# cbouilla/spasm

Hardware: AMD Instinct MI355X
Metric: rows eliminated/sec (sparse Schur complement, mod 42013) (higher is better)
Workload: dtype i32 sums of i16 x i16 products

## Files before the change

spasm_amd/csrc/backsolve.hip:

```cpp
#include <algorithm>
#include <cinttypes>
#include <type_traits>
#include <thread>
#include <vector>

#include "device_types.h"
#include "field_dev.h"
#include "sgn_dev.h"

namespace sh {

int usable_cpus();

namespace {

constexpr int BS_RING = 768;
constexpr int BS_NEARCAP = 1024;
constexpr int BS_PASSCAP = 80;
constexpr int BS_PASSROWS = 32;
constexpr uint32_t BS_NONE = 0xFFFFFFFFu;

template <typename T> T *dalloc(int64_t count)
{
	return static_cast<T *>(sh::big_alloc((size_t) (count > 0 ? count : 1) * sizeof(T)));
// ... 1187 lines not shown
					dst[u] = at;
					if (v0[u] != 0)
						cbuf[at] = qq[u].x;
					if (v1[u] != 0)
						cbuf[at + (v0[u] != 0 ? 1u : 0u)] = qq[u].y;
					gpos += (uint32_t) (__popcll(m0) + __popcll(m1));
				}
				for (uint32_t t = lane; t < gpos; t += 64)
					oj[wpos + t] = cbuf[t];
#pragma unroll
				for (int u = 0; u < AP_TU; u++) {
					if (v0[u] != 0)
						cbuf[dst[u]] = v0[u];
					if (v1[u] != 0)
						cbuf[dst[u] + (v0[u] != 0 ? 1u : 0u)] = v1[u];
				}
				for (uint32_t t = lane; t < gpos; t += 64)
					ox[wpos + t] = cbuf[t];
				wpos += gpos;
			};
			constexpr int GW = 64 * AP_TU;
			issue(0, qa);
			issue(GW, qb);
			for (int t0 = 0; t0 < nwords; t0 += 3 * GW) {
				issue(t0 + 2 * GW, qc);
				emit(t0, qa);
				issue(t0 + 3 * GW, qa);
				if (t0 + GW < nwords)
					emit(t0 + GW, qb);
				issue(t0 + 4 * GW, qb);
				if (t0 + 2 * GW < nwords)
					emit(t0 + 2 * GW, qc);
			}
		}
		st_done += fits ? 1 : 0;
		k0 = k1;
		c0 = c1;
		k1 = -1;
		uint32_t *const t = x0;
		x0 = x1;
		x1 = t;
		return true;
	};

	for (;;) {
		if (k0 >= 0)
			settle(k1 >= 0);
		const int k = next_ticket(d, lane);
		if (k >= a.nrows)
			break;
		uint32_t *xw = (k0 < 0) ? x0 : x1;
		const int i = a.rows[k];
		const int64_t lo = a.Ap[i], hi = a.Ap[i + 1];
		st_input += (unsigned long long) (hi - lo);
		int count = s16_reduce_segment<true>(d, F, G, lo, hi, 0, nwords, plist, xw, lane, true, st_piv);
		if (count < 0) {
			count = 0;
			for (int t0 = 0; t0 < nwords; t0 += 64) {
				const uint32_t w = xw[t0 + lane];
				count += __popcll(__ballot((w & 0xFFFFu) != 0)) + __popcll(__ballot((w >> 16) != 0));
			}
		}
		if (lane == 0)
			__hip_atomic_store(&d.status[k], LB_FLAG_LEN | (unsigned long long) count, __ATOMIC_RELAXED, __HIP_MEMORY_SCOPE_AGENT);
		if (k0 < 0) {
			k0 = k;
			c0 = count;
		} else {
			k1 = k;
			c1 = count;
		}
	}
	while (k0 >= 0)
		settle(true);
	if (lane == 0) {
		if (lost)
			atomicOr(&a.ctr[CTR_STATUS], 4);
		atomicAdd(&a.ctr64[C64_INPUT], st_input);
		atomicAdd(&a.ctr64[C64_ELIM], st_piv);
		atomicAdd(&a.ctr[a.done_ctr], st_done);
	}
}

constexpr int SCAN_BLOCK = 1024;

__global__ __launch_bounds__(SCAN_BLOCK) void bs_scan_lengths_kernel(const int *len, int n, const unsigned long long *block_sum, int64_t *Sp, int64_t cap,
                                                                      int *ctr)
{
	__shared__ long long part[SCAN_BLOCK / 64];
	__shared__ long long s_base;
	const int tid = threadIdx.x, lane = tid & 63, wave = tid >> 6;
	const int g = blockIdx.x;
	auto wave_sum = [](long long v) -> long long {
		for (int sft = 32; sft >= 1; sft >>= 1) {
			const uint32_t lo32 = (uint32_t) __shfl_xor((int) (uint32_t) v, sft);
			const uint32_t hi32 = (uint32_t) __shfl_xor((int) (uint32_t) ((unsigned long long) v >> 32), sft);
			v += (long long) (((unsigned long long) hi32 << 32) | lo32);
		}
		return v;
	};
	long long before = 0;
	for (int b = tid; b < g; b += SCAN_BLOCK)
		before += (long long) block_sum[b];
	before = wave_sum(before);
	if (lane == 0)
		part[wave] = before;
	__syncthreads();
	if (tid == 0) {
		long long t = Sp[0];
		for (int w = 0; w < SCAN_BLOCK / 64; w++)
			t += part[w];
		s_base = t;
	}
	__syncthreads();
	const long long base = s_base;
	__syncthreads();
	const int k = g * SCAN_BLOCK + tid;
	const long long mine = (k < n) ? (long long) len[k] : 0;
	long long incl = mine;
	for (int sft = 1; sft < 64; sft <<= 1) {
		const uint32_t lo32 = (uint32_t) __shfl_up((int) (uint32_t) incl, sft);
		const uint32_t hi32 = (uint32_t) __shfl_up((int) (uint32_t) ((unsigned long long) incl >> 32), sft);
		if (lane >= sft)
			incl += (long long) (((unsigned long long) hi32 << 32) | lo32);
	}
	if (lane == 63)
		part[wave] = incl;
	__syncthreads();
	long long waves_before = 0;
	for (int w = 0; w < wave; w++)
		waves_before += part[w];
	const long long end = base + waves_before + incl;
	if (k < n) {
		Sp[k + 1] = end;
		if (k == n - 1 && end > cap)
			atomicOr(&ctr[CTR_STATUS], 1);
	}
}

struct ExpandArgs {
	const uint32_t *stage;
	int nwords, nrows;
	const int64_t *Sp;
	int *Sj, *Sx;
	int64_t cap;
	const int *q;
	SgnDev G;
};


template <int FMT> __global__ __launch_bounds__(256) void bs_expand_kernel(ExpandArgs e)
{
	constexpr int TU = 4;
	__shared__ int stage_j[4][128 * TU], stage_x[4][128 * TU];
	const int lane = threadIdx.x & 63, wv = threadIdx.x >> 6;
	const int wave = (int) ((blockIdx.x * blockDim.x + threadIdx.x) >> 6), nwaves = (int) ((gridDim.x * blockDim.x) >> 6);
	const int2 *q2 = reinterpret_cast<const int2 *>(e.q) + lane;
	const int *q1 = e.q + lane;
	const SgnDev G = e.G;
	const uint32_t pu = (uint32_t) G.p, halfu = (uint32_t) G.half;
	auto balanced = [&](uint32_t v) -> int { return (v > halfu) ? (int) (v - pu) : (int) v; };
	const int last = e.nwords - 64 * TU;
	int *sj = stage_j[wv], *sx = stage_x[wv];
	for (int k = wave; k < e.nrows; k += nwaves) {
		const int64_t off = e.Sp[k], end = e.Sp[k + 1];
		if (end > e.cap || end == off)
// ... 707 lines not shown
	}
	b.sparse_init = (B.nnp <= 4 * (int64_t) B.r && env_int("SPASM_HIP_BS_SPARSE_INIT", 1) != 0) ? 1 : 0;
	HIP_CHECK(hipEventRecord(B.ev0, stream));
	if (fresh || !b.sparse_init)
		HIP_CHECK(hipMemsetAsync(B.d_R, 0, bytes, stream));
	if (!b.sparse_init) {
		if (packed)
			hipLaunchKernelGGL(bs_init_kernel<uint16_t>, dim3((B.r + 255) / 256), dim3(256), 0, stream, b);
		else
			hipLaunchKernelGGL(bs_init_kernel<uint32_t>, dim3((B.r + 255) / 256), dim3(256), 0, stream, b);
	}
	const int shape = B.shape;
	if (shape == 3)
		snprintf(B.kernel_build, sizeof(B.kernel_build), "backsolve_kernel<true,true,8,8,true,768,64,31,2>");
	else if (shape == 4)
		snprintf(B.kernel_build, sizeof(B.kernel_build), "backsolve_kernel<true,true,10,10,true,1260,64,48,1>");
	else if (shape == 5)
		snprintf(B.kernel_build, sizeof(B.kernel_build), "backsolve_kernel<true,true,12,12,true,1200,64,44,1>");
	else
		snprintf(B.kernel_build, sizeof(B.kernel_build), "backsolve_kernel<%s,%s,%d,%d,%s,%d,%d,%d,1>", packed ? "true" : "false", B.plain ? "true" : "false",
		         shape == 2 ? 16 : 32, (shape == 0 || (!packed && B.plain && shape == 1)) ? 16 : 8, B.sgn ? "true" : "false", BS_RING, BS_PASSROWS,
		         BS_PASSCAP);
	if (B.sgn) {
		if (shape == 3)
			launch_backsolve_variant<true, true, 8, 8, true, 768, 64, 31, 2>(b, B.Sm, stream, B);
		else if (shape == 4)
			launch_backsolve_variant<true, true, 10, 10, true, 1260, 64, 48, 1>(b, B.Sm, stream, B);
		else if (shape == 5)
			launch_backsolve_variant<true, true, 12, 12, true, 1200, 64, 44, 1>(b, B.Sm, stream, B);
		else if (shape == 1)
			launch_backsolve_variant<true, true, 32, 8, true>(b, B.Sm, stream, B);
		else if (shape == 2)
			launch_backsolve_variant<true, true, 16, 8, true>(b, B.Sm, stream, B);
		else
			launch_backsolve_variant<true, true, 32, 16, true>(b, B.Sm, stream, B);
	} else if (packed) {
		if (shape == 1)
			launch_backsolve_variant<true, true, 32, 8>(b, B.Sm, stream, B);
		else if (shape == 2)
			launch_backsolve_variant<true, true, 16, 8>(b, B.Sm, stream, B);
		else
			launch_backsolve_variant<true, true, 32, 16>(b, B.Sm, stream, B);
	} else if (B.plain) {
		if (shape == 2)
			launch_backsolve_variant<false, true, 16, 8>(b, B.Sm, stream, B);
		else
			launch_backsolve_variant<false, true, 32, 16>(b, B.Sm, stream, B);
	} else {
		if (shape == 1)
			launch_backsolve_variant<false, false, 32, 8>(b, B.Sm, stream, B);
		else if (shape == 2)
			launch_backsolve_variant<false, false, 16, 8>(b, B.Sm, stream, B);
		else
			launch_backsolve_variant<false, false, 32, 16>(b, B.Sm, stream, B);
	}
	HIP_CHECK(hipGetLastError());
	HIP_CHECK(hipEventRecord(B.ev1, stream));
	B.valid = true;
	B.builds += 1;
	if (b.prof != nullptr) {
		unsigned long long h[8];
		HIP_CHECK(hipMemcpyAsync(h, b.prof, sizeof(h), hipMemcpyDeviceToHost, stream));
		HIP_CHECK(hipStreamSynchronize(stream));
		static const char *const stage[7] = {"descriptor + metadata issue", "phase A", "non-pivotal entries added", "long outside lists", "phase B", "phase C",
		                                     "metadata into LDS"};
		unsigned long long tot = 0;
		for (int q = 0; q < 7; q++)
			tot += h[q];
		fprintf(stderr, "[bs profile] %s, %d chunks, workgroup 0, shader-clock cycles per chunk:", B.kernel_build, B.nchunks);
		for (int q = 0; q < 7; q++)
			fprintf(stderr, " %s %.0f (%.0f%%);", stage[q], (double) h[q] / B.nchunks, 100.0 * (double) h[q] / (double) (tot ? tot : 1));
		fprintf(stderr, " total %.0f\n", (double) tot / B.nchunks);
		sh::big_free(b.prof);
	}
}

bool backsolve_stages_output(const spasm_hip_dfact *F, int64_t *row_bytes)
{
	const BsImage &B = F->bs;
	*row_bytes = B.ldR * (B.valid ? B.elem_bytes : 4);
	return B.planned && env_int("SPASM_HIP_BS_STAGED", 1) != 0;
}

static size_t csr_wave_bytes(int64_t ldR)
{
	return (size_t) CSR_SCRATCH_BYTES + 2 * (size_t) ldR * 2;
}

bool backsolve_output_csr(const spasm_hip_dfact *F, int64_t nrows, int64_t stage_rows)
{
	const BsImage &B = F->bs;
	if (!B.valid || !B.sgn || B.ldR > 24576 || stage_rows < nrows || env_int("SPASM_HIP_BS_CSR", 1) == 0)
		return false;
	int dev = 0, per_block = 0;
	HIP_CHECK(hipGetDevice(&dev));
	HIP_CHECK(hipDeviceGetAttribute(&per_block, hipDeviceAttributeMaxSharedMemoryPerBlock, dev));
	return csr_wave_bytes(B.ldR) <= (size_t) per_block;
}

void launch_backsolve_apply(const SchurArgs &a, const spasm_hip_dfact *F, uint32_t *dense_out, int64_t ldS, hipStream_t stream,
                            BsDirectOut *direct)
{
	const BsImage &B = F->bs;
	if (!B.valid)
		die("launch_backsolve_apply: R has not been built");
	ApplyArgs d{};
	d.a = a;
	d.R = B.d_R;
	d.ldR = B.ldR;
	d.col = B.d_col;
	d.r = B.r;
	static_assert(2 * 64 * AP_TU == 512, "ldR is padded to whole tile groups of the apply kernels");
	d.Smpad = (int) B.ldR;
	d.dense_out = dense_out;
	d.ldS = ldS;
	d.sgn = B.sgn ? 1 : 0;
	d.G = sgn_setup(F->prime);
	if (direct != nullptr && dense_out == nullptr) {
		d.direct = 1;
		d.status = direct->status;
		d.ticket = direct->ticket;
		d.Sp = direct->Sp;
		d.Sj = direct->Sj;
		d.Sx = direct->Sx;
		d.cap = direct->cap;
	}
	const bool packed = B.elem_bytes == 2;
	int dev = 0;
	HIP_CHECK(hipGetDevice(&dev));
	hipDeviceProp_t prop;
	HIP_CHECK(hipGetDeviceProperties(&prop, dev));
	if (dense_out != nullptr && a.nrows > 0 && a.nrows < prop.multiProcessorCount && a.avg_row_entries >= 1024) {
		const int nwords = d.Smpad / (packed ? 2 : 1);
		const dim3 grid((unsigned) ((nwords + 64 * AP_TU - 1) / (64 * AP_TU)), (unsigned) a.nrows);
		if (packed)
			hipLaunchKernelGGL((bs_apply_wide_kernel<true, true>), grid, dim3(64 * AW_NW), 0, stream, d);
		else if (B.plain)
			hipLaunchKernelGGL((bs_apply_wide_kernel<false, true>), grid, dim3(64 * AW_NW), 0, stream, d);
		else
			hipLaunchKernelGGL((bs_apply_wide_kernel<false, false>), grid, dim3(64 * AW_NW), 0, stream, d);
		HIP_CHECK(hipGetLastError());
		return;
	}
	if (direct != nullptr && direct->csr && dense_out == nullptr) {
		const size_t per_wave = csr_wave_bytes(B.ldR);
		int per_block = 0;
		HIP_CHECK(hipDeviceGetAttribute(&per_block, hipDeviceAttributeMaxSharedMemoryPerBlock, dev));
		int waves = 1, best = 0;
		for (int w = 1; w <= 8 && (size_t) w * per_wave <= (size_t) per_block; w++) {
			const int fit = (int) ((size_t) (160 * 1024) / ((size_t) w * per_wave)) * w;
			if (fit >= best) {
				best = fit;
				waves = w;
			}
		}
		d.waves = waves;
		d.wave_bytes = per_wave;
		d.seg_words = d.Smpad / 2;
		const size_t lds = per_wave * (size_t) waves;
		static size_t configured = 0;
		if (lds > configured) {
			HIP_CHECK(hipFuncSetAttribute(reinterpret_cast<const void *>(&bs_apply_s16_csr_kernel), hipFuncAttributeMaxDynamicSharedMemorySize, (int) lds));
			configured = lds;
		}
		int per_cu = 0;
		HIP_CHECK(hipOccupancyMaxActiveBlocksPerMultiprocessor(&per_cu, bs_apply_s16_csr_kernel, 64 * waves, lds));
		per_cu = std::min(per_cu, (int) ((size_t) (160 * 1024) / lds));
		if (per_cu < 1)
			die("launch_backsolve_apply: %zu bytes of LDS per workgroup leave no room for the CSR output", lds);
		const int blocks = std::max(1, std::min((a.nrows + waves - 1) / waves, prop.multiProcessorCount * per_cu));
		d.ntickets = std::min(LB_TICKETS, blocks);
		if (verbose() >= 3)
			logmsg("[dense image] CSR output: %d workgroups of %d waves, %zu bytes of LDS each, %d per CU\n", blocks, waves, lds, per_cu);
		hipLaunchKernelGGL(bs_apply_s16_csr_kernel, dim3(blocks), dim3(64 * waves), lds, stream, d);
		HIP_CHECK(hipGetLastError());
		return;
	}
	const bool staged_call = direct != nullptr && direct->stage != nullptr && dense_out == nullptr;
	int seg_cols = d.Smpad;
	if (B.sgn && d.Smpad > 24576 && (staged_call || dense_out != nullptr))
		seg_cols = 8192;
	d.seg_words = seg_cols / 2;
	const size_t per_wave = ((size_t) seg_cols * (size_t) B.elem_bytes + (size_t) AP_LIST * sizeof(uint2) + 15) / 16 * 16;
	if (per_wave > 150 * 1024)
		die("launch_backsolve_apply: %d non-pivotal columns do not fit the LDS row buffer", B.Sm);
	const int waves = (int) std::max<size_t>(1, std::min<size_t>(8, (size_t) (76 * 1024) / per_wave));
	d.waves = waves;
	d.wave_bytes = per_wave;
	const size_t lds = per_wave * (size_t) waves;
	int blocks = std::max(1, std::min((a.nrows + waves - 1) / waves, prop.multiProcessorCount * 8));
	if (d.direct) {
		const int per_cu = (int) std::max<size_t>(1, (size_t) (160 * 1024) / std::max<size_t>(lds, 1));
		blocks = std::min(blocks, prop.multiProcessorCount * per_cu);
	}
	d.ntickets = std::min(LB_TICKETS, blocks);
	auto launch_apply = [&](const ApplyArgs &dd, int nblocks_apply) {
		if (B.sgn) {
			static size_t configured = 0;
			if (lds > configured) {
				HIP_CHECK(hipFuncSetAttribute(reinterpret_cast<const void *>(&bs_apply_s16_kernel), hipFuncAttributeMaxDynamicSharedMemorySize, (int) lds));
				configured = lds;
			}
			hipLaunchKernelGGL(bs_apply_s16_kernel, dim3(nblocks_apply), dim3(64 * dd.waves), lds, stream, dd);
		} else if (packed) {
			launch_apply_variant<true, true>(dd, nblocks_apply, lds, stream);
		} else if (B.plain) {
			launch_apply_variant<false, true>(dd, nblocks_apply, lds, stream);
		} else {
			launch_apply_variant<false, false>(dd, nblocks_apply, lds, stream);
		}
	};
	if (direct != nullptr && direct->stage != nullptr && dense_out == nullptr) {
		const int nwords = d.Smpad / (packed ? 2 : 1);
		HIP_CHECK(hipMemsetAsync(direct->Sp, 0, sizeof(int64_t), stream));
		auto expand_slice = [&](int64_t r0, int n, const uint32_t *stage, const unsigned long long *block_sum, hipStream_t s2) {
			const int nblocks = (n + SCAN_BLOCK - 1) / SCAN_BLOCK;
			hipLaunchKernelGGL(bs_scan_lengths_kernel, dim3(nblocks), dim3(SCAN_BLOCK), 0, s2, a.row_len + r0, n, block_sum, direct->Sp + r0, direct->cap, a.ctr);
			ExpandArgs e{stage, nwords, n, direct->Sp + r0, direct->Sj, direct->Sx, direct->cap, a.q, d.G};
			const int blocks3 = std::max(1, std::min((n + 3) / 4, prop.multiProcessorCount * 8));
			if (B.sgn)
				hipLaunchKernelGGL(bs_expand_kernel<0>, dim3(blocks3), dim3(256), 0, s2, e);
			else if (packed)
				hipLaunchKernelGGL(bs_expand_kernel<1>, dim3(blocks3), dim3(256), 0, s2, e);
			else
				hipLaunchKernelGGL(bs_expand_kernel<2>, dim3(blocks3), dim3(256), 0, s2, e);
		};
		for (int64_t r0 = 0; r0 < a.nrows; r0 += direct->stage_rows) {
			const int n = (int) std::min<int64_t>(direct->stage_rows, a.nrows - r0);
			ApplyArgs d2 = d;
			d2.direct = 0;
			d2.stage = direct->stage;
			d2.a.rows = a.rows + r0;
			d2.a.row_len = a.row_len + r0;
			d2.a.nrows = n;
			const int blocks2 = std::max(1, std::min((n + waves - 1) / waves, prop.multiProcessorCount * 8));
			const int nblocks = (n + SCAN_BLOCK - 1) / SCAN_BLOCK;
			d2.block_sum = direct->status;
			HIP_CHECK(hipMemsetAsync(d2.block_sum, 0, (size_t) nblocks * sizeof(unsigned long long), stream));
			launch_apply(d2, blocks2);
			if (direct->ev_expand != nullptr)
				HIP_CHECK(hipEventRecord(direct->ev_expand, stream));
			expand_slice(r0, n, direct->stage, d2.block_sum, stream);
			direct->staged = true;
			direct->slices += 1;
		}
	} else {
		launch_apply(d, blocks);
	}
	HIP_CHECK(hipGetLastError());
}

}
```

spasm_amd/csrc/device_types.h:

```cpp
#pragma once

#include <hip/hip_runtime.h>

#include <cstdint>
#include <memory>
#include <vector>

#include "common.h"

namespace sh {

#define HIP_CHECK(expr)                                                                                  \
	do {                                                                                             \
		hipError_t e_ = (expr);                                                                  \
		if (e_ != hipSuccess)                                                                    \
			sh::die("%s failed: %s (%s:%d)", #expr, hipGetErrorString(e_), __FILE__, __LINE__); \
	} while (0)

struct MontDev {
	uint32_t p, pinv, r1, r2, half;
};

inline MontDev to_dev(const Mont &M) { return MontDev{M.p, M.pinv, M.r1, M.r2, M.half}; }

// ... 147 lines not shown
struct SpPending;
struct SpImage {
	std::shared_ptr<SpPending> pending;
	int pending_m = 0;
	bool planned = false;
	bool valid = false;
	bool failed = false;
	bool wide = false;
	int r = 0, Sm = 0, nseg = 0, nlevels = 0;
	int64_t ndeps = 0, nnp = 0;
	std::vector<int> lvl_lo;
	int *d_col = nullptr;
	uint64_t *d_dep_rp = nullptr;
	uint2 *d_dep = nullptr;
	uint64_t *d_np_rp = nullptr;
	uint2 *d_np = nullptr;
	uint64_t *d_segmask = nullptr;
	uint2 *d_head = nullptr;
	uint64_t *d_rowmask = nullptr;
	uint64_t *d_frag = nullptr;
	uint32_t *d_chunk[SP_MAX_CHUNKS] = {};
	int64_t chunk_cap[SP_MAX_CHUNKS] = {};
	int nchunks = 0;
	unsigned long long *d_shard = nullptr;
	unsigned long long *d_stat = nullptr;
	hipEvent_t ev0 = nullptr, ev1 = nullptr;
	int builds = 0;
	int64_t nnz = 0;
	int64_t ops_build = 0;
	int64_t pool_used = 0;
	int launches = 0;
};

struct SchurArgs;
struct FactPlan;
void launch_map_columns(int *d_Sj, int64_t nnz, const int *d_cols, hipStream_t stream);
void comm_allreduce_min_i32(struct ::spasm_hip_comm *c, int *d_buf, int64_t count, hipStream_t stream);
void comm_allreduce_sum_i32(struct ::spasm_hip_comm *c, int *d_buf, int64_t count, hipStream_t stream);
void comm_allreduce_sum_u32(struct ::spasm_hip_comm *c, uint32_t *d_buf, int64_t count, hipStream_t stream);
int comm_allgatherv_csr(struct ::spasm_hip_comm *c, int my_rows, int64_t my_nnz, const int64_t *own_Sp, const int *own_Sj, const int *own_Sx, int64_t *d_Sp, int *d_Sj,
                        int *d_Sx, int64_t cap, int *total_rows, int64_t *total_nnz, hipStream_t stream);
void launch_stitch_slabs(const int64_t *gSp, const int *gSj, const int *gSx, int n, int parts, int64_t *Sp, int *Sj, int *Sx, int64_t cap, int *d_len,
                         unsigned long long *d_block_sum, int *d_ctr, hipStream_t stream);
void launch_scan_lengths(const int *len, int n, const unsigned long long *block_sum, int64_t *Sp, int64_t cap, int *ctr, hipStream_t stream);

struct DeviceMatrix {
	int64_t *p = nullptr;
	int *j = nullptr, *x = nullptr;
	int64_t nnz = 0;
	bool owned = false;
	DeviceMatrix(const struct spasm_csr *A, hipStream_t stream, bool slab_will_do = false);
	~DeviceMatrix();
	DeviceMatrix(const DeviceMatrix &) = delete;
	DeviceMatrix &operator=(const DeviceMatrix &) = delete;
};
void *big_alloc(size_t bytes);
void big_free(void *ptr);
void big_trim(size_t keep_bytes = 0);
void h2d(void *dst, const void *src, size_t bytes, hipStream_t stream);
void d2h(void *dst, const void *src, size_t bytes, hipStream_t stream);
void big_age(int max_idle);
hipError_t malloc_or_trim(void **ptr, size_t bytes);
void mem_info(size_t *free_b, size_t *total_b);
void resident_adopt_slab(const struct spasm_csr *host, int64_t *dp, int *dj, int *dx, int64_t local_nnz, struct ::spasm_hip_comm *comm);
struct ::spasm_hip_comm *resident_slab_comm(const struct spasm_csr *A);
void resident_begin();
void resident_end();
void resident_forget(const struct spasm_csr *A);
bool resident_enabled();
void resident_prefetch(const struct spasm_csr *A);
void ensure_row_tables(const struct ::spasm_hip_dfact *F, hipStream_t stream, bool components = true);
void resident_counters(int64_t *uploads, int64_t *hits);
void resident_lazy_downloads(bool on);
void resident_materialize(const struct spasm_csr *A);
int resident_fl_census(const struct spasm_csr *A);

struct BsDirectOut {
	unsigned long long *status;
	int *ticket;
	int64_t *Sp;
	int *Sj, *Sx;
	int64_t cap;
	bool csr = false;
	uint32_t *stage = nullptr;
	int64_t stage_rows = 0;
	hipEvent_t ev_expand = nullptr;
	bool staged = false;
	int slices = 0;
};

}

struct spasm_hip_dfact {
	int m = 0, r = 0, Sm = 0, nlevels = 0;
	int rpad = 0;
	mutable bool row_tables = false;
	mutable int maxdeg = 0;
	mutable int ncomp = 0, comp_largest = 0;
	int64_t nnz = 0;
	int64_t prime = 0;
	sh::Mont mont{};
	uint32_t *d_lab = nullptr;
	int *d_q = nullptr;
	uint64_t *d_rp = nullptr;
	uint2 *d_ent = nullptr;
	uint2 *d_head = nullptr;
	mutable uint32_t *d_comp = nullptr;
	uint32_t *d_lvl_end = nullptr;
	uint32_t *d_lvl_end_w = nullptr;
	int *d_kof = nullptr;
	uint64_t *d_cp = nullptr;
	uint2 *d_cent = nullptr;
	int2 *d_lvl = nullptr;
	bool has_pull = false;
	std::vector<int> h_q;
	std::vector<int> h_kof;
	mutable sh::BsImage bs;
	mutable sh::SpImage sp;
	mutable bool bs_deferred = false;
	mutable std::unique_ptr<sh::FactPlan> host_plan;
};

struct spasm_hip_dwork {
	int max_rows = 0, m = 0;
	int64_t pool_cap = 0;
	int *d_pool_j = nullptr, *d_pool_x = nullptr;
	int64_t *d_row_off = nullptr;
	int *d_row_len = nullptr;
	int *d_ovf1 = nullptr, *d_ovf2 = nullptr;
	int *d_ctr = nullptr;
	unsigned long long *d_ctr64 = nullptr;
	int64_t *d_Sp = nullptr;
	int64_t *d_blocksum = nullptr;
	int *d_order = nullptr, *d_sortbuf = nullptr;
	int64_t sortbuf_ints = 0;
	int *d_Sj = nullptr, *d_Sx = nullptr;
	uint32_t *d_stage = nullptr;
	int64_t stage_bytes = 0;
	uint64_t *d_spT = nullptr;
	int64_t spT_words = 0;
	unsigned long long *d_lb_status = nullptr;
	unsigned char *d_scratch = nullptr;
	int64_t scratch_bytes = 0;
	int64_t scratch_budget = 0;
	int scratch_slots = 0;
	int64_t slot_bytes = 0, off_bm = 0, off_xn = 0;
	hipEvent_t ev[7] = {nullptr, nullptr, nullptr, nullptr, nullptr, nullptr, nullptr};
	int last_rows = 0;
	int64_t last_nnz = 0;
};
```

spasm_amd/csrc/schur_api.hip:

```cpp
#include <algorithm>
#include <unordered_map>
#include <atomic>
#include <thread>
#include <cinttypes>
#include <mutex>
#include <vector>

#include "device_types.h"

namespace sh {
void launch_schur_lds(const SchurArgs &a, int table, bool wide, int blocks, hipStream_t stream);
size_t schur_lds_bytes(int table, bool wide);
void launch_finalize(const spasm_hip_dwork *W, int nrows, hipStream_t stream);
void wave_dense_geometry(int rpad, int Sm, bool wide, int64_t *slot_bytes, int64_t *off_bm, int64_t *off_xn);
void group_geometry(int rpad, int Sm, bool wide, int64_t *slot_bytes, int64_t *off_bm);
int64_t regroup_scratch_ints(int nrows, int r);
void launch_regroup_rows(const SchurArgs &a, int *sortbuf, int *order, hipStream_t stream);
void launch_schur_group(const SchurArgs &a, unsigned char *scratch, int64_t slot_bytes, int64_t off_bm, bool wide,
                        uint32_t *dense_out, int64_t ldS, int blocks, hipStream_t stream, int watch, float min_eff,
                        long long min_w, int waves);
void launch_schur_wave_dense(const SchurArgs &a, unsigned char *scratch, int64_t slot_bytes, int64_t off_bm, int64_t off_xn,
                             bool wide, uint32_t *dense_out, int64_t ldS, int blocks, hipStream_t stream);
void launch_all_rows_to_list(int *list, int *count, int *row_len, int nrows, hipStream_t stream);
void schur_group_variant_name(int r, bool wide, int waves, char *out, size_t cap);
// ... 1613 lines not shown
		int slots = cus * 32;
		size_t free_b = 0, total_b = 0;
		sh::mem_info(&free_b, &total_b);
		i64 budget = (i64) ((free_b + (size_t) W->scratch_bytes) / 2);
		if (W->scratch_budget > 0)
			budget = std::min(budget, std::max(W->scratch_budget, W->scratch_bytes));
		if (env_int("SPASM_HIP_SCRATCH_GB", 0) > 0)
			budget = (i64) env_int("SPASM_HIP_SCRATCH_GB", 0) << 30;
		slots = (int) std::max<i64>(cus, std::min<i64>(slots, budget / slot_bytes));
		slots = std::max(1, std::min(slots, nrows));
		i64 need = slot_bytes * slots;
		if (group_mode) {
			group_geometry(F->rpad, F->Sm, wide_dense, &group_slot_bytes, &group_off_bm);
			const int ngroups = (nrows + 63) / 64;
			const i64 slices_that_fit = budget / group_slot_bytes;
			if (slices_that_fit < 1 || (slices_that_fit < std::min<i64>(ngroups, cus / 2) && env_int("SPASM_HIP_GROUP", -1) < 0)) {
				group_mode = 0;
				probe = false;
			}
		}
		if (group_mode) {
			const int ngroups = (nrows + 63) / 64;
			const i64 in_flight = std::min<i64>(ngroups, budget / group_slot_bytes);
			group_waves = env_int("SPASM_HIP_GROUP_WAVES", in_flight <= cus * 3 ? 4 : in_flight <= cus * 12 ? 2 : 1);
			group_slots = (int) std::min<i64>((group_waves >= 4 ? cus * 2 : group_waves >= 2 ? cus * 4 : cus * 8),
			                                  budget / group_slot_bytes);
			group_slots = std::max(1, std::min(group_slots, ngroups));
			need = probe ? std::max(need, group_slot_bytes * group_slots) : group_slot_bytes * group_slots;
		}
		if (need > W->scratch_bytes) {
			if (W->d_scratch != nullptr)
				sh::big_free(W->d_scratch);
			HIP_CHECK(sh::malloc_or_trim((void **) &W->d_scratch, (size_t) need));
			W->scratch_bytes = need;
			HIP_CHECK(hipMemsetAsync(W->d_scratch, 0, (size_t) need, stream));
		} else if (slot_bytes != W->slot_bytes || off_bm != W->off_bm || off_xn != W->off_xn) {
		}
		W->scratch_slots = slots;
		W->slot_bytes = slot_bytes;
		W->off_bm = off_bm;
		W->off_xn = off_xn;
	}

	HIP_CHECK(hipMemsetAsync(W->d_ctr, 0, CTR_COUNT * sizeof(int), stream));
	HIP_CHECK(hipMemsetAsync(W->d_ctr64, 0, C64_COUNT * sizeof(unsigned long long), stream));
	HIP_CHECK(hipEventRecord(W->ev[0], stream));

	SchurArgs a{};
	a.Ap = A->p;
	a.Aj = A->j;
	a.Ax = A->x;
	a.rows = d_rows;
	a.nrows = nrows;
	a.lab = F->d_lab;
	a.q = F->d_q;
	a.rp = F->d_rp;
	a.ent = F->d_ent;
	a.head = F->d_head;
	a.comp = F->d_comp;
	a.lvl_end = F->d_lvl_end;
	a.lvl_end_w = F->d_lvl_end_w;
	a.r = F->rpad;
	a.Sm = F->m - F->r;
	a.m = F->m;
	a.F = to_dev(F->mont);
	a.pool_j = W->d_pool_j;
	a.pool_x = W->d_pool_x;
	a.pool_cap = W->pool_cap;
	a.row_off = W->d_row_off;
	a.row_len = W->d_row_len;
	a.ctr = W->d_ctr;
	a.ctr64 = W->d_ctr64;
	if (Lout != nullptr) {
		a.L_i = Lout->Li;
		a.L_j = Lout->Lj;
		a.L_x = Lout->Lx;
		a.L_cap = Lout->cap;
		a.kof = F->d_kof;
		a.row_orig = Lout->row_orig;
	}

	bool used_bs = false, built_bs = false, bs_direct = false, use_pull = false;
	int bs_staged_slices = 0;
	if (want_sp) {
		group_mode = 0;
		HIP_CHECK(hipEventRecord(W->ev[5], stream));
		a.list = nullptr;
		a.list_count = nullptr;
		a.done_ctr = CTR_DONE2;
		bs_direct = true;
		const i64 twords = sparse_image_table_words(nrows, F->sp.nseg);
		if (W->spT_words < twords) {
			if (W->d_spT != nullptr)
				sh::big_free(W->d_spT);
			W->d_spT = dalloc<uint64_t>(twords);
			W->spT_words = twords;
		}
		if (W->d_lb_status == nullptr)
			W->d_lb_status = dalloc<unsigned long long>((i64) W->max_rows + 16 + 16 * 16);
		launch_sparse_image_apply(a, F, reinterpret_cast<uint32_t *>(W->d_pool_j), reinterpret_cast<uint32_t *>(W->d_pool_x), W->pool_cap, W->d_spT, W->d_lb_status, W->d_Sp, W->d_Sj,
		                          W->d_Sx, W->pool_cap, stream, W->ev[6]);
		HIP_CHECK(hipEventRecord(W->ev[3], stream));
		HIP_CHECK(hipEventRecord(W->ev[4], stream));
		goto eliminated;
	}
	if (want_bs) {
		used_bs = true;
		group_mode = 0;
		if (!F->bs.valid) {
			backsolve_build(F, stream);
			built_bs = true;
		}
		HIP_CHECK(hipEventRecord(W->ev[5], stream));
		a.list = nullptr;
		a.list_count = nullptr;
		a.done_ctr = CTR_DONE2;
		bs_direct = env_int("SPASM_HIP_BS_DIRECT", 1) != 0;
		if (bs_direct) {
			if (W->d_lb_status == nullptr)
				W->d_lb_status = dalloc<unsigned long long>((i64) W->max_rows + 16 + 16 * 16);
			const size_t ticket_at = ((size_t) nrows + 16) / 16 * 16;
			HIP_CHECK(hipMemsetAsync(W->d_lb_status, 0, (ticket_at + 16 * 16) * sizeof(unsigned long long), stream));
			BsDirectOut out{W->d_lb_status, reinterpret_cast<int *>(W->d_lb_status + ticket_at), W->d_Sp, W->d_Sj, W->d_Sx, W->pool_cap};
			int64_t stage_row_bytes = 0;
			if (backsolve_stages_output(F, &stage_row_bytes) && nrows > 0) {
				const int64_t budget = (int64_t) env_int("SPASM_HIP_STAGE_GB", 8) << 30;
				int64_t rows_fit = std::max<int64_t>(1024, budget / stage_row_bytes);
				if (env_int("SPASM_HIP_STAGE_ROWS", 0) > 0)
					rows_fit = env_int("SPASM_HIP_STAGE_ROWS", 0);
				out.stage_rows = std::min<int64_t>(nrows, rows_fit);
				if (backsolve_output_csr(F, nrows, out.stage_rows)) {
					out.csr = true;
				} else {
					const int64_t need = out.stage_rows * stage_row_bytes;
					if (W->stage_bytes < need) {
						if (W->d_stage != nullptr)
							sh::big_free(W->d_stage);
						W->d_stage = dalloc<uint32_t>(need / 4);
						W->stage_bytes = need;
					}
					out.stage = W->d_stage;
					out.ev_expand = W->ev[6];
				}
			}
			launch_backsolve_apply(a, F, nullptr, 0, stream, &out);
			bs_staged_slices = out.staged ? out.slices : 0;
		} else {
			launch_backsolve_apply(a, F, nullptr, 0, stream, nullptr);
		}
		HIP_CHECK(hipEventRecord(W->ev[3], stream));
		HIP_CHECK(hipEventRecord(W->ev[4], stream));
		goto eliminated;
	}
	if (nrows > 0) {
		a.list = nullptr;
		a.list_count = nullptr;
		a.ovf_list = W->d_ovf1;
		a.next_ctr = CTR_ROW_NEXT;
		a.ovf_ctr = CTR_OVF1;
		a.done_ctr = CTR_DONE0;
		const int per_cu0 = (int) std::min<size_t>(16, (size_t) (160 * 1024) / schur_lds_bytes(small_table, wide_lds));
		int blocks0 = std::min(cus * per_cu0, (nrows + 3) / 4);
		if (group_mode) {
			a.next_ctr = CTR_ROW_NEXT_G;
			a.done_ctr = CTR_DONE2;
			HIP_CHECK(hipMemsetAsync(W->d_row_len, 0xFF, (size_t) nrows * sizeof(int), stream));
			const float min_eff = (float) (4) / 100.0f;
			const char *min_w_env = sh::env_get("SPASM_HIP_GROUP_MIN_PIVOTS");
			const long long min_w = (min_w_env != nullptr) ? std::atoll(min_w_env) : std::max<long long>(500000, 8192ll * group_slots);
			const bool regroup_enabled = env_int("SPASM_HIP_GROUP_REGROUP", 1) != 0;
			auto regroup = [&]() {
				const int64_t need = regroup_scratch_ints(nrows, F->rpad);
				if (W->sortbuf_ints < need) {
					if (W->d_sortbuf != nullptr)
						sh::big_free(W->d_sortbuf);
					W->d_sortbuf = dalloc<int>(need);
					W->sortbuf_ints = need;
				}
				if (W->d_order == nullptr)
					W->d_order = dalloc<int>(W->max_rows);
				launch_regroup_rows(a, W->d_sortbuf, W->d_order, stream);
			};
			const bool grouped_first = regroup_enabled && F->ncomp > 1 && Lout == nullptr &&
			                           (i64) F->comp_largest * 10 < (i64) F->r * 9;
			if (grouped_first) {
				regroup();
				a.order = W->d_order;
			}
			use_pull = Lout == nullptr && env_int("SPASM_HIP_PULL", 0) != 0 && F->has_pull && pull_lds_bytes(F->rpad, F->Sm) <= (size_t) 150 * 1024;
			if (use_pull) {
				const int per_cu = (int) std::max<size_t>(1, std::min<size_t>(8, (size_t) (160 * 1024) / (pull_lds_bytes(F->rpad, F->Sm) + 5 * 1024)));
				const int pull_slots = (int) std::max<i64>(1, std::min<i64>(std::min<i64>((nrows + 63) / 64, (i64) cus * per_cu),
				                                                          W->scratch_bytes / pull_slot_bytes(F->rpad, F->Sm)));
				probe = false;
				launch_schur_pull(a, W->d_scratch, pull_slot_bytes(F->rpad, F->Sm), F->d_cp, F->d_cent, F->d_lvl, F->nlevels, pull_slots, stream);
			} else
			launch_schur_group(a, W->d_scratch, group_slot_bytes, group_off_bm, wide_dense, nullptr, 0, group_slots, stream,
			                   probe ? 1 : 0, min_eff, min_w, group_waves);
			a.order = nullptr;
			a.skip_ctr = CTR_GROUP_ABORT;
			int gave_up = 0;
			if (probe) {
				HIP_CHECK(hipMemcpyAsync(&gave_up, W->d_ctr + CTR_GROUP_ABORT, sizeof(int), hipMemcpyDeviceToHost, stream));
				HIP_CHECK(hipStreamSynchronize(stream));
			}
			HIP_CHECK(hipEventRecord(W->ev[5], stream));
			if (!probe || !gave_up) {
				HIP_CHECK(hipEventRecord(W->ev[3], stream));
				HIP_CHECK(hipEventRecord(W->ev[4], stream));
				goto eliminated;
			}
			a.skip_done = 1;
			a.next_ctr = CTR_ROW_NEXT;
			a.done_ctr = CTR_DONE0;
		}
		if (force_tier == 0)
			launch_schur_lds(a, small_table, wide_lds, std::max(blocks0, 1), stream);
		else
			launch_all_rows_to_list(W->d_ovf1, W->d_ctr + CTR_OVF1, W->d_row_len, nrows, stream);
		HIP_CHECK(hipEventRecord(W->ev[3], stream));
		const int *last_list = W->d_ovf1;
		const int *last_count = W->d_ctr + CTR_OVF1;
		if (use_big) {
			a.list = W->d_ovf1;
			a.list_count = W->d_ctr + CTR_OVF1;
			a.ovf_list = W->d_ovf2;
			a.next_ctr = CTR_ROW_NEXT2;
			a.ovf_ctr = CTR_OVF2;
			a.done_ctr = CTR_DONE1;
// ... 35 lines not shown
	const int status = ctr[CTR_STATUS] & 3;
#ifdef SPASM_GROUP_PROFILE
	if (group_mode) {
		static const char *const phase[8] = {"drain", "watch", "bitmap scan", "level end", "gather pending", "apply+scatter", "output count", "output write"};
		const double g = (double) ((nrows + 63) / 64);
		for (int q = 0; q < 8; q++)
			fprintf(stderr, "[spasm_hip profile] %-15s %12.0f per group\n", phase[q], (double) ctr64[C64_PROF0 + q] / g);
	}
#endif
	if (Lout != nullptr)
		Lout->used = (i64) ctr64[C64_LPOOL];
	if (stats != nullptr) {
		stats->nnz = total;
		stats->eliminations = (i64) ctr64[C64_ELIM];
		stats->entries_streamed = (i64) ctr64[C64_STREAM];
		stats->input_entries = (i64) ctr64[C64_INPUT];
		stats->group_pivots = (i64) ctr64[C64_WAVEPIV];
		stats->used_group_kernel = group_mode ? 1 : 0;
		stats->group_slots = group_mode ? group_slots : 0;
		stats->group_waves = group_mode ? group_waves : 0;
		stats->group_slot_bytes = group_mode ? group_slot_bytes : 0;
		stats->group_slots_wanted = group_mode ? (int) std::min<i64>((nrows + 63) / 64, (i64) cus * 8 / std::max(1, group_waves)) : 0;
		stats->rows = nrows;
		stats->rows_lds = ctr[CTR_DONE0];
		stats->rows_lds_big = ctr[CTR_DONE1];
		stats->rows_dense = ctr[CTR_DONE2];
		stats->status = status;
		HIP_CHECK(hipEventElapsedTime(&stats->ms_eliminate, W->ev[0], W->ev[1]));
		stats->ms_tier0 = stats->ms_tier1 = stats->ms_tier2 = stats->ms_group = 0.0f;
		stats->group_aborted = ctr[CTR_GROUP_ABORT] ? 1 : 0;
		stats->used_backsolve = used_bs ? 1 : 0;
		stats->backsolve_built = built_bs ? 1 : 0;
		stats->ms_backsolve = stats->ms_apply = 0.0f;
		stats->bytes_backsolve = stats->bytes_apply = 0;
		stats->kernel[0] = 0;
		stats->kernel_other[0] = 0;
		stats->kernel_expand[0] = 0;
		stats->ms_expand = stats->ms_pad = 0.0f;
		stats->bytes_expand = stats->bytes_staged = 0;
		stats->used_sparse_image = want_sp ? 1 : 0;
		stats->sparse_image_built = built_sp ? 1 : 0;
		stats->ms_sparse_build = stats->ms_sparse_apply = stats->ms_sparse_gather = 0.0f;
		stats->sparse_image_nnz = stats->sparse_image_ops_build = stats->sparse_image_ops_apply = 0;
		stats->sparse_image_levels = stats->sparse_image_launches = 0;
		stats->bytes_sparse_build = stats->bytes_sparse_apply = stats->bytes_sparse_gather = 0;
		if (want_sp) {
			const SpImage &P = F->sp;
			if (built_sp)
				HIP_CHECK(hipEventElapsedTime(&stats->ms_sparse_build, P.ev0, P.ev1));
			HIP_CHECK(hipEventElapsedTime(&stats->ms_sparse_apply, W->ev[5], W->ev[6]));
			HIP_CHECK(hipEventElapsedTime(&stats->ms_sparse_gather, W->ev[6], W->ev[1]));
			stats->sparse_image_nnz = P.nnz;
			stats->sparse_image_ops_build = P.ops_build;
			stats->sparse_image_ops_apply = (i64) ctr64[C64_STREAM];
			stats->sparse_image_levels = P.nlevels;
			stats->sparse_image_launches = P.launches;
			stats->bytes_sparse_build = 4 * (P.ops_build + P.nnz) + 8 * (P.ndeps + (i64) P.r) * P.nseg + 8 * F->nnz;
			stats->bytes_sparse_apply = 4 * (i64) ctr64[C64_STREAM] + 8 * (i64) ctr64[C64_ELIM] * P.nseg + 8 * (i64) ctr64[C64_INPUT] + 4 * total +
			                            8 * (i64) nrows * P.nseg;
			stats->bytes_sparse_gather = 12 * total + 8 * (i64) nrows * P.nseg + 8 * (i64) nrows;
			const bool build_dominates = stats->ms_sparse_build > stats->ms_sparse_apply;
			snprintf(stats->kernel, sizeof(stats->kernel), "%s", build_dominates ? "sp_build_kernel" : "sp_apply_kernel");
			snprintf(stats->kernel_other, sizeof(stats->kernel_other), "%s", build_dominates ? "sp_apply_kernel" : "sp_build_kernel");
			snprintf(stats->kernel_expand, sizeof(stats->kernel_expand), "sp_gather_kernel");
		} else if (used_bs) {
			const BsImage &B = F->bs;
			if (built_bs) {
				HIP_CHECK(hipEventElapsedTime(&stats->ms_backsolve, B.ev0, B.ev1));
				stats->bytes_backsolve = ((i64) B.r + B.ndeps) * (i64) B.Sm * B.elem_bytes + 8 * F->nnz;
			}
			HIP_CHECK(hipEventElapsedTime(&stats->ms_apply, W->ev[5], W->ev[1]));
			stats->bytes_apply = (i64) ctr64[C64_ELIM] * (i64) B.Sm * B.elem_bytes + 8 * ((i64) ctr64[C64_INPUT] + total) + 20 * (i64) nrows;
			if (bs_staged_slices > 0) {
				stats->bytes_apply -= 8 * total;
				stats->bytes_expand = 8 * total;
				stats->bytes_staged = (i64) nrows * B.ldR * B.elem_bytes;
				snprintf(stats->kernel_expand, sizeof(stats->kernel_expand), "bs_expand_kernel<%d>", B.sgn ? 0 : B.elem_bytes == 2 ? 1 : 2);
				if (bs_staged_slices == 1) {
					HIP_CHECK(hipEventElapsedTime(&stats->ms_apply, W->ev[5], W->ev[6]));
					HIP_CHECK(hipEventElapsedTime(&stats->ms_expand, W->ev[6], W->ev[1]));
				}
			}
			char apply_name[32];
			if (B.sgn)
				snprintf(apply_name, sizeof(apply_name), "bs_apply_s16_kernel");
			else
				snprintf(apply_name, sizeof(apply_name), "bs_apply_kernel<%s,%s>", B.elem_bytes == 2 ? "true" : "false", B.plain ? "true" : "false");
			const bool build_dominates = stats->ms_backsolve > stats->ms_apply;
			snprintf(stats->kernel, sizeof(stats->kernel), "%s", build_dominates ? B.kernel_build : apply_name);
			snprintf(stats->kernel_other, sizeof(stats->kernel_other), "%s", build_dominates ? apply_name : B.kernel_build);
		} else if (group_mode && use_pull) {
			snprintf(stats->kernel, sizeof(stats->kernel), "schur_pull_kernel");
		} else if (group_mode && !stats->group_aborted) {
			schur_group_variant_name(F->rpad, wide_dense, group_waves, stats->kernel, sizeof(stats->kernel));
		} else {
			snprintf(stats->kernel, sizeof(stats->kernel), "schur_wave_dense_kernel<%s>", wide_dense ? "true" : "false");
		}
		if (nrows > 0 && !used_bs && !want_sp) {
			if (group_mode)
				HIP_CHECK(hipEventElapsedTime(&stats->ms_group, W->ev[0], W->ev[5]));
			HIP_CHECK(hipEventElapsedTime(&stats->ms_tier0, group_mode ? W->ev[5] : W->ev[0], W->ev[3]));
			HIP_CHECK(hipEventElapsedTime(&stats->ms_tier1, W->ev[3], W->ev[4]));
			HIP_CHECK(hipEventElapsedTime(&stats->ms_tier2, W->ev[4], W->ev[1]));
		}
		HIP_CHECK(hipEventElapsedTime(&stats->ms_finalize, W->ev[1], W->ev[2]));
		HIP_CHECK(hipEventElapsedTime(&stats->ms_total, W->ev[0], W->ev[2]));
		if (built_sp) {
			stats->ms_total += stats->ms_sparse_build;
			stats->ms_eliminate += stats->ms_sparse_build;
		}
	}
	return status;
}
}

extern "C" {

int spasm_hip_dschur(const spasm_hip_dcsr *A, const int *d_rows, int nrows, const spasm_hip_dfact *F,
                     spasm_hip_dwork *W, void *stream, spasm_hip_schur_stats *stats)
{
	return dschur_impl(A, d_rows, nrows, F, W, stream, stats, nullptr);
}

void spasm_hip_dschur_row_pointers(const spasm_hip_dwork *W, i64 *d_Sp, void *stream_)
{
	hipStream_t stream = (hipStream_t) stream_;
	HIP_CHECK(hipMemcpyAsync(d_Sp, W->d_Sp, ((size_t) W->last_rows + 1) * sizeof(i64), hipMemcpyDefault, stream));
}

void spasm_hip_dschur_fetch(const spasm_hip_dwork *W, i64 *d_Sp, int *d_Sj, spasm_ZZp *d_Sx, void *stream_)
{
	hipStream_t stream = (hipStream_t) stream_;
	HIP_CHECK(hipMemcpyAsync(d_Sp, W->d_Sp, ((size_t) W->last_rows + 1) * sizeof(i64), hipMemcpyDefault, stream));
	if (W->last_nnz > 0) {
		HIP_CHECK(hipMemcpyAsync(d_Sj, W->d_Sj, (size_t) W->last_nnz * sizeof(int), hipMemcpyDefault, stream));
		HIP_CHECK(hipMemcpyAsync(d_Sx, W->d_Sx, (size_t) W->last_nnz * sizeof(int), hipMemcpyDefault, stream));
	}
	HIP_CHECK(hipStreamSynchronize(stream));
}

extern "C" {
static struct spasm_csr *schur_entry(const struct spasm_csr *A, const int *p, int n, const struct spasm_lu *fact, double est_density, struct spasm_triplet *L,
                                     const int *p_in, int *p_out, spasm_hip_dwork **keep_on_device);
}

static struct spasm_csr *schur_by_column_slabs(const struct spasm_csr *A, const int *p, int n, const struct spasm_lu *fact, double est_density,
                                               const int *p_in, int *p_out, spasm_hip_comm *comm)
{
	const double t0 = wtime();
	const int m = A->m, world = comm_world(comm), rank = comm_rank(comm);
	const i64 prime = A->field->p;
	hipStream_t stream = nullptr;
	struct spasm_csr *A_slab = nullptr;
	struct spasm_lu *F_slab = nullptr;
	std::vector<int> cols((size_t) (m > 0 ? m : 1));
	const int mm = spasm_hip_column_slab(A, fact, rank, world, &A_slab, &F_slab, cols.data());
	const double t_slab = wtime() - t0;
	spasm_hip_dwork *W = nullptr;
	(void) schur_entry(A_slab, p, n, F_slab, est_density, nullptr, nullptr, nullptr, &W);
	const i64 snz = W->last_nnz;
	int *d_cols = dalloc<int>(mm);
	upload(d_cols, cols.data(), mm, stream);
	launch_map_columns(W->d_Sj, snz, d_cols, stream);
	HIP_CHECK(hipStreamSynchronize(stream));
	resident_forget(A_slab);
	spasm_hip_csr_free(A_slab);
	spasm_hip_lu_free(F_slab);
// ... 350 lines not shown
```

Baseline: 36.34 million.

## Hold pending CSR row in registers to halve per-wave LDS buffers

Adds a templated CSR-output apply kernel that copies the finished row from LDS into a register file before the next row is reduced. Each wave then needs one LDS row buffer instead of two, so more waves fit per CU for rows up to 40 tiles. The launcher now picks the wave count from occupancy queries per candidate. The cost is much higher register pressure, many template instantiations, and an extra LDS-to-register copy per row.

```diff
diff --git a/spasm_amd/csrc/backsolve.hip b/spasm_amd/csrc/backsolve.hip
--- a/spasm_amd/csrc/backsolve.hip
+++ b/spasm_amd/csrc/backsolve.hip
@@ -1293,6 +1293,163 @@
 	}
 }
 
+constexpr int CSR_ROWREG_MAX_TILES = 40;
+constexpr bool CSR_ROWREG_DEEP = false;
+constexpr int CSR_ROWREG_WPE = 4;
+
+template <int NT, bool DEEP, int WPE>
+__global__ __launch_bounds__(512, WPE) void bs_apply_s16_csr_rowreg_kernel(ApplyArgs d)
+{
+	static_assert(NT % AP_TU == 0 && NT >= AP_TU && NT <= CSR_ROWREG_MAX_TILES, "whole tile groups");
+	extern __shared__ __attribute__((aligned(16))) unsigned char lds_raw[];
+	const SchurArgs &a = d.a;
+	const int lane = threadIdx.x & 63, wave = threadIdx.x >> 6;
+	const MontDev F = a.F;
+	const SgnDev G = d.G;
+	constexpr int nwords = 64 * NT;
+	constexpr int NG = NT / AP_TU;
+	constexpr int GW = 64 * AP_TU;
+	unsigned char *area = lds_raw + (size_t) wave * d.wave_bytes;
+	uint2 *plist = reinterpret_cast<uint2 *>(area);
+	int *cbuf = reinterpret_cast<int *>(area);
+	uint32_t *xl = reinterpret_cast<uint32_t *>(area + CSR_SCRATCH_BYTES);
+	unsigned long long st_input = 0, st_piv = 0;
+	int st_done = 0;
+	bool lost = false;
+	RegFile<uint32_t, NT> xr;
+	int k0 = -1, c0 = 0, k1 = -1, c1 = 0;
+
+	auto settle = [&](bool wait) -> bool {
+		unsigned long long end = 0;
+		if (!lookback_probe(d, k0, lane, wait, end, lost))
+			return false;
+		const int64_t off = (int64_t) (end - (unsigned long long) c0);
+		const bool fits = !lost && end <= (unsigned long long) d.cap;
+		if (lane == 0) {
+			d.Sp[k0] = off;
+			if (k0 == a.nrows - 1)
+				d.Sp[a.nrows] = (int64_t) end;
+			if (!fits)
+				atomicOr(&a.ctr[CTR_STATUS], 1);
+		}
+		if (fits && c0 > 0) {
+			int *oj = d.Sj + off, *ox = d.Sx + off;
+			uint32_t wpos = 0;
+			int2 qa[AP_TU], qb[AP_TU], qc[AP_TU];
+			auto issue = [&](int t0, int2 (&qq)[AP_TU]) {
+				uint32_t at = (uint32_t) (t0 + lane) * (uint32_t) sizeof(int2);
+				asm volatile("" : "+v"(at));
+				const int2 *qg = reinterpret_cast<const int2 *>(reinterpret_cast<const char *>(a.q) + at);
+#pragma unroll
+				for (int u = 0; u < AP_TU; u++)
+					qq[u] = qg[64 * u];
+			};
+			auto emit = [&](auto gg, const int2 (&qq)[AP_TU]) {
+				constexpr int g = decltype(gg)::value;
+				int v0[AP_TU], v1[AP_TU];
+				uint32_t dst[AP_TU], gpos = 0;
+				bs_static_for<0, AP_TU>([&](auto uu) {
+					constexpr int u = decltype(uu)::value;
+					sgn_unpack(xr.template at<g * AP_TU + u>(), v0[u], v1[u]);
+					v0[u] = sgn_canonical(v0[u], G);
+					v1[u] = sgn_canonical(v1[u], G);
+					const uint64_t m0 = __ballot(v0[u] != 0), m1 = __ballot(v1[u] != 0);
+					uint32_t at = gpos;
+					at = __builtin_amdgcn_mbcnt_hi((uint32_t) (m0 >> 32), __builtin_amdgcn_mbcnt_lo((uint32_t) m0, at));
+					at = __builtin_amdgcn_mbcnt_hi((uint32_t) (m1 >> 32), __builtin_amdgcn_mbcnt_lo((uint32_t) m1, at));
+					dst[u] = at;
+					if (v0[u] != 0)
+						cbuf[at] = qq[u].x;
+					if (v1[u] != 0)
+						cbuf[at + (v0[u] != 0 ? 1u : 0u)] = qq[u].y;
+					gpos += (uint32_t) (__popcll(m0) + __popcll(m1));
+				});
+				for (uint32_t t = lane; t < gpos; t += 64)
+					oj[wpos + t] = cbuf[t];
+#pragma unroll
+				for (int u = 0; u < AP_TU; u++) {
+					if (v0[u] != 0)
+						cbuf[dst[u]] = v0[u];
+					if (v1[u] != 0)
+						cbuf[dst[u] + (v0[u] != 0 ? 1u : 0u)] = v1[u];
+				}
+				for (uint32_t t = lane; t < gpos; t += 64)
+					ox[wpos + t] = cbuf[t];
+				wpos += gpos;
+			};
+			issue(0, qa);
+			if constexpr (NG > 1)
+				issue(GW, qb);
+			bs_static_for<0, NG>([&](auto gg) {
+				constexpr int g = decltype(gg)::value;
+				if constexpr (g % 3 == 0) {
+					if constexpr (g + 2 < NG)
+						issue((g + 2) * GW, qc);
+					emit(gg, qa);
+				} else if constexpr (g % 3 == 1) {
+					if constexpr (g + 2 < NG)
+						issue((g + 2) * GW, qa);
+					emit(gg, qb);
+				} else {
+					if constexpr (g + 2 < NG)
+						issue((g + 2) * GW, qb);
+					emit(gg, qc);
+				}
+			});
+		}
+		st_done += fits ? 1 : 0;
+		k0 = -1;
+		return true;
+	};
+	auto hand_over = [&]() {
+		bs_static_for<0, NT>([&](auto tt) {
+			constexpr int t = decltype(tt)::value;
+			xr.template at<t>() = xl[64 * t + lane];
+		});
+		k0 = k1;
+		c0 = c1;
+		k1 = -1;
+	};
+
+	for (bool finishing = false;;) {
+		if (k1 >= 0 && k0 < 0)
+			hand_over();
+		if (k0 >= 0)
+			settle(k1 >= 0 || finishing);
+		if (k1 >= 0)
+			hand_over();
+		if (finishing)
+			break;
+		const int k = next_ticket(d, lane);
+		if (k >= a.nrows) {
+			finishing = true;
+			continue;
+		}
+		const int i = a.rows[k];
+		const int64_t lo = a.Ap[i], hi = a.Ap[i + 1];
+		st_input += (unsigned long long) (hi - lo);
+		int count = s16_reduce_segment<DEEP>(d, F, G, lo, hi, 0, nwords, plist, xl, lane, true, st_piv);
+		if (count < 0) {
+			count = 0;
+			for (int t0 = 0; t0 < nwords; t0 += 64) {
+				const uint32_t w = xl[t0 + lane];
+				count += __popcll(__ballot((w & 0xFFFFu) != 0)) + __popcll(__ballot((w >> 16) != 0));
+			}
+		}
+		if (lane == 0)
+			__hip_atomic_store(&d.status[k], LB_FLAG_LEN | (unsigned long long) count, __ATOMIC_RELAXED, __HIP_MEMORY_SCOPE_AGENT);
+		k1 = k;
+		c1 = count;
+	}
+	if (lane == 0) {
+		if (lost)
+			atomicOr(&a.ctr[CTR_STATUS], 4);
+		atomicAdd(&a.ctr64[C64_INPUT], st_input);
+		atomicAdd(&a.ctr64[C64_ELIM], st_piv);
+		atomicAdd(&a.ctr[a.done_ctr], st_done);
+	}
+}
+
 constexpr int SCAN_BLOCK = 1024;
 
 __global__ __launch_bounds__(SCAN_BLOCK) void bs_scan_lengths_kernel(const int *len, int n, const unsigned long long *block_sum, int64_t *Sp, int64_t cap,
@@ -2166,9 +2323,30 @@
 	return B.planned && env_int("SPASM_HIP_BS_STAGED", 1) != 0;
 }
 
-static size_t csr_wave_bytes(int64_t ldR)
-{
-	return (size_t) CSR_SCRATCH_BYTES + 2 * (size_t) ldR * 2;
+static size_t csr_wave_bytes(int64_t ldR, int buffers)
+{
+	return (size_t) CSR_SCRATCH_BYTES + (size_t) buffers * (size_t) ldR * 2;
+}
+
+static int csr_rowreg_tiles(int64_t ldR)
+{
+	if (ldR > 128 * CSR_ROWREG_MAX_TILES || env_int("SPASM_HIP_BS_CSR_ROWREG", 1) == 0)
+		return 0;
+	return (int) (ldR / 128);
+}
+
+using CsrKernel = void (*)(ApplyArgs);
+static CsrKernel csr_kernel(int tiles)
+{
+	switch (tiles) {
+	case 0: return bs_apply_s16_csr_kernel;
+#define ROWREG_CASE(NT) case NT: return bs_apply_s16_csr_rowreg_kernel<NT, CSR_ROWREG_DEEP, CSR_ROWREG_WPE>;
+	ROWREG_CASE(4) ROWREG_CASE(8) ROWREG_CASE(12) ROWREG_CASE(16) ROWREG_CASE(20)
+	ROWREG_CASE(24) ROWREG_CASE(28) ROWREG_CASE(32) ROWREG_CASE(36) ROWREG_CASE(40)
+#undef ROWREG_CASE
+	}
+	die("launch_backsolve_apply: no CSR-output kernel for rows of %d tiles", tiles);
+	return nullptr;
 }
 
 bool backsolve_output_csr(const spasm_hip_dfact *F, int64_t nrows, int64_t stage_rows)
@@ -2179,7 +2357,7 @@
 	int dev = 0, per_block = 0;
 	HIP_CHECK(hipGetDevice(&dev));
 	HIP_CHECK(hipDeviceGetAttribute(&per_block, hipDeviceAttributeMaxSharedMemoryPerBlock, dev));
-	return csr_wave_bytes(B.ldR) <= (size_t) per_block;
+	return csr_wave_bytes(B.ldR, csr_rowreg_tiles(B.ldR) > 0 ? 1 : 2) <= (size_t) per_block;
 }
 
 void launch_backsolve_apply(const SchurArgs &a, const spasm_hip_dfact *F, uint32_t *dense_out, int64_t ldS, hipStream_t stream,
@@ -2227,14 +2405,22 @@
 		return;
 	}
 	if (direct != nullptr && direct->csr && dense_out == nullptr) {
-		const size_t per_wave = csr_wave_bytes(B.ldR);
+		const int tiles = csr_rowreg_tiles(B.ldR);
+		const CsrKernel kernel = csr_kernel(tiles);
+		const size_t per_wave = csr_wave_bytes(B.ldR, tiles > 0 ? 1 : 2);
 		int per_block = 0;
 		HIP_CHECK(hipDeviceGetAttribute(&per_block, hipDeviceAttributeMaxSharedMemoryPerBlock, dev));
-		int waves = 1, best = 0;
-		for (int w = 1; w <= 8 && (size_t) w * per_wave <= (size_t) per_block; w++) {
-			const int fit = (int) ((size_t) (160 * 1024) / ((size_t) w * per_wave)) * w;
-			if (fit >= best) {
-				best = fit;
+		const int max_waves = (int) std::min<size_t>(8, (size_t) per_block / per_wave);
+		HIP_CHECK(hipFuncSetAttribute(reinterpret_cast<const void *>(kernel), hipFuncAttributeMaxDynamicSharedMemorySize,
+		                              (int) (per_wave * (size_t) max_waves)));
+		int waves = 1, per_cu = 0;
+		for (int w = 1; w <= max_waves; w++) {
+			const size_t lds_w = per_wave * (size_t) w;
+			int fit = 0;
+			HIP_CHECK(hipOccupancyMaxActiveBlocksPerMultiprocessor(&fit, kernel, 64 * w, lds_w));
+			fit = std::min(fit, (int) ((size_t) (160 * 1024) / lds_w));
+			if (fit * w >= per_cu * waves) {
+				per_cu = fit;
 				waves = w;
 			}
 		}
@@ -2242,21 +2428,15 @@
 		d.wave_bytes = per_wave;
 		d.seg_words = d.Smpad / 2;
 		const size_t lds = per_wave * (size_t) waves;
-		static size_t configured = 0;
-		if (lds > configured) {
-			HIP_CHECK(hipFuncSetAttribute(reinterpret_cast<const void *>(&bs_apply_s16_csr_kernel), hipFuncAttributeMaxDynamicSharedMemorySize, (int) lds));
-			configured = lds;
-		}
-		int per_cu = 0;
-		HIP_CHECK(hipOccupancyMaxActiveBlocksPerMultiprocessor(&per_cu, bs_apply_s16_csr_kernel, 64 * waves, lds));
-		per_cu = std::min(per_cu, (int) ((size_t) (160 * 1024) / lds));
 		if (per_cu < 1)
 			die("launch_backsolve_apply: %zu bytes of LDS per workgroup leave no room for the CSR output", lds);
 		const int blocks = std::max(1, std::min((a.nrows + waves - 1) / waves, prop.multiProcessorCount * per_cu));
 		d.ntickets = std::min(LB_TICKETS, blocks);
+		direct->csr_tiles = tiles;
 		if (verbose() >= 3)
-			logmsg("[dense image] CSR output: %d workgroups of %d waves, %zu bytes of LDS each, %d per CU\n", blocks, waves, lds, per_cu);
-		hipLaunchKernelGGL(bs_apply_s16_csr_kernel, dim3(blocks), dim3(64 * waves), lds, stream, d);
+			logmsg("[dense image] CSR output (%s): %d workgroups of %d waves, %zu bytes of LDS each, %d per CU\n",
+			       tiles > 0 ? "pending row in registers" : "two row buffers", blocks, waves, lds, per_cu);
+		hipLaunchKernelGGL(kernel, dim3(blocks), dim3(64 * waves), lds, stream, d);
 		HIP_CHECK(hipGetLastError());
 		return;
 	}
diff --git a/spasm_amd/csrc/device_types.h b/spasm_amd/csrc/device_types.h
--- a/spasm_amd/csrc/device_types.h
+++ b/spasm_amd/csrc/device_types.h
@@ -253,6 +253,7 @@
 	int *Sj, *Sx;
 	int64_t cap;
 	bool csr = false;
+	int csr_tiles = -1;
 	uint32_t *stage = nullptr;
 	int64_t stage_rows = 0;
 	hipEvent_t ev_expand = nullptr;
diff --git a/spasm_amd/csrc/schur_api.hip b/spasm_amd/csrc/schur_api.hip
--- a/spasm_amd/csrc/schur_api.hip
+++ b/spasm_amd/csrc/schur_api.hip
@@ -1719,6 +1719,7 @@
 
 	bool used_bs = false, built_bs = false, bs_direct = false, use_pull = false;
 	int bs_staged_slices = 0;
+	int bs_csr_tiles = -1;
 	if (want_sp) {
 		group_mode = 0;
 		HIP_CHECK(hipEventRecord(W->ev[5], stream));
@@ -1782,6 +1783,7 @@
 			}
 			launch_backsolve_apply(a, F, nullptr, 0, stream, &out);
 			bs_staged_slices = out.staged ? out.slices : 0;
+			bs_csr_tiles = out.csr_tiles;
 		} else {
 			launch_backsolve_apply(a, F, nullptr, 0, stream, nullptr);
 		}
@@ -1983,7 +1985,9 @@
 				}
 			}
 			char apply_name[32];
-			if (B.sgn)
+			if (B.sgn && bs_csr_tiles == 0)
+				snprintf(apply_name, sizeof(apply_name), "bs_apply_s16_kernel<lds2>");
+			else if (B.sgn)
 				snprintf(apply_name, sizeof(apply_name), "bs_apply_s16_kernel");
 			else
 				snprintf(apply_name, sizeof(apply_name), "bs_apply_kernel<%s,%s>", B.elem_bytes == 2 ? "true" : "false", B.plain ? "true" : "false");
```

Result: faster. 40.61 million (median of 6 runs) (+11.8%).
